# xinntao/EDVR

Hardware: AMD Instinct MI355X
Metric: EDVR-L x4 5-frame 720p clips/sec (higher is better)
Workload: dtype fp32 emulated as 2xf16 (hi+lo, 22-bit operands, 4 cross products), fp32 accumulate; 1 GPU; EDVR-L x4, 5 frames, 180x320 LR -> 720x1280, batch 10/GPU, inference; clips_per_gpu=10, global_clips=10, parallelism=clip-sharded x1, no data-path collective, world_size=1, backend=single process

## Files before the change

edvr_amd/_lib.py:

```python
import ctypes
import os

_HERE = os.path.dirname(os.path.abspath(__file__))
LIB_PATH = os.environ.get('EDVR_AMD_LIB') or os.path.join(_HERE, 'lib', 'libedvr_amd.so')

c_float_p = ctypes.c_void_p
i32, i64, f32, sz = ctypes.c_int, ctypes.c_int64, ctypes.c_float, ctypes.c_size_t
vp = ctypes.c_void_p


class ConvDesc(ctypes.Structure):
    _fields_ = [
        ('x1', vp), ('x2', vp), ('c1', i32), ('c2', i32), ('x1_img_stride', i64), ('x2_img_stride', i64),
        ('x2_div', i32), ('x2_mul', i32), ('x2_add', i32), ('n', i32), ('h', i32), ('w', i32), ('wpk', vp),
        ('bias', vp), ('co', i32), ('ks', i32), ('stride', i32), ('act', i32), ('act_from', i32), ('res1', vp),
        ('res2', vp), ('res1_img_stride', i64), ('res2_img_stride', i64), ('y', vp), ('y_img_stride', i64),
        ('out_mode', i32), ('algo', i32), ('gate', vp), ('gate_img_stride', i64), ('gate_slope', f32), ('y_scale', f32),
        ('wpk_f4', vp), ('abs_sum', vp), ('abs_sum_channels', i32), ('wpk_f4s', vp), ('x_amax', vp), ('y_amax', vp),
        ('pre', vp), ('pre_img_stride', i64), ('pre_div', i32), ('pre_mul', i32), ('pre_add', i32), ('pre_n', i32),
    ]


PROTOTYPES = {
    'edvr_version': (ctypes.c_char_p, []),
    'edvr_last_error': (ctypes.c_char_p, []),
    'edvr_check_device': (i32, []),
    'edvr_conv2d_packed_weight_elems': (sz, [i32, i32, i32]),
    'edvr_conv2d_pack_weight_f32': (i32, [vp, vp, i32, i32, i32, i32, vp]),
    'edvr_conv2d_packed_weight_f4_elems': (sz, [i32, i32]),
    'edvr_conv2d_pack_weight_f4_f32': (i32, [vp, vp, i32, i32, i32, vp]),
    'edvr_conv2d_packed_weight_f4s_elems': (sz, [i32, i32]),
    'edvr_conv2d_pack_weight_f4s_f32': (i32, [vp, vp, i32, i32, i32, vp]),
    'edvr_conv2d_packed_weight_1x1s_elems': (sz, [i32, i32]),
    'edvr_conv2d_pack_weight_1x1s_f32': (i32, [vp, vp, i32, i32, vp]),
    'edvr_amax_f32': (i32, [vp, vp, i32, i64, i64, vp]),
    'edvr_pack_job_bytes': (sz, []),
    'edvr_conv2d_pack_weights_multi': (i32, [vp, i32, i32, i32, vp]),
    'edvr_conv2d_f32': (i32, [ctypes.POINTER(ConvDesc), vp]),
    'edvr_conv2d_gate_supported': (i32, [ctypes.POINTER(ConvDesc)]),
    'edvr_conv2d_abs_sum_supported': (i32, [ctypes.POINTER(ConvDesc)]),
    'edvr_conv2d_y_amax_supported': (i32, [ctypes.POINTER(ConvDesc)]),
    'edvr_conv2d_pre_supported': (i32, [ctypes.POINTER(ConvDesc)]),
    'edvr_conv2d_kernel_name': (i32, [ctypes.POINTER(ConvDesc), ctypes.c_char_p, sz]),
    'edvr_conv2d_executed_flops': (i32, [ctypes.POINTER(ConvDesc), ctypes.POINTER(ctypes.c_double)]),
    'edvr_dcnv2_fwd_ws_bytes': (sz, [i32] * 12),
    'edvr_dcnv2_fwd_f32': (i32, [vp] * 6 + [i32] * 12 + [i64, i64, i32, i32, vp, sz, vp]),
    'edvr_dcnv2_fwd_split_f32': (i32, [vp] * 6 + [i32] * 12 + [i64, i64, i32, i32, vp, sz, vp, vp]),
    'edvr_dcnv2_fwd_split_applies': (i32, [vp] + [i32] * 13),
    'edvr_dcnv2_fwd_kernel_name': (i32, [vp] + [i32] * 13 + [ctypes.c_char_p, sz]),
    'edvr_dcnv2_bwd_ws_bytes': (sz, [i32] * 12),
    'edvr_dcnv2_any_ws_bytes': (sz, [i32] * 13),
    'edvr_dcnv2_fwd_any': (i32, [i32] + [vp] * 6 + [i32] * 12 + [i64, i64, vp, sz, vp]),
    'edvr_dcnv2_bwd_any': (i32, [i32] + [vp] * 10 + [i32] * 12 + [i64, i64, i64, i64, vp, sz, vp]),
    'edvr_psnr_sse_f32': (i32, [vp, vp, vp, i32, i32, i32, i32, i64, i64, i32, i32, i32, vp]),
    'edvr_ssim_partials': (sz, [i32, i32, i32]),
    'edvr_ssim_f32': (i32, [vp, vp, vp, i32, i32, i32, i32, i64, i64, i32, i32, vp]),
    'edvr_niqe_blocks': (sz, [i32, i32, i32]),
    'edvr_niqe_moments_f32': (i32, [vp, vp, i32, i32, i32, i32, i64, i32, vp]),
    'edvr_niqe_moments_u8': (i32, [vp, vp, i32, i32, i32, i64, i32, vp]),
    'edvr_frames_u8_to_f32': (i32, [vp, vp, i32, i32, i32, i32, vp, i32, vp]),
    'edvr_gather_images_f32': (i32, [vp, vp, vp, vp, i32, vp, i32, i32, vp]),
    'edvr_upsample4x_add_u8': (i32, [vp, vp, vp, i32, i32, i32, vp]),
    'edvr_f32_to_u8_hwc': (i32, [vp, vp, i32, i32, i32, i64, vp]),
    'edvr_crop_pad_frames_u8': (i32, [vp, vp, i32, i32, i32, i32, i32, i32, i32, i32, vp]),
    'edvr_crop_pad_frames_f32': (i32, [vp, vp, i32, i32, i32, i64, i32, i32, i32, i32, i32, vp]),
    'edvr_upsample4x_add_rect_f32': (i32, [vp, vp, vp, i32, i32, i32, i32, i32, i32, i32, i64, i64, i64, vp]),
    'edvr_upsample4x_add_rect_u8': (i32, [vp, vp, vp, i32, i32, i32, i32, i32, i32, i32, i64, i64, vp]),
    'edvr_f32_to_u8_hwc_rect': (i32, [vp, vp, i32, i32, i32, i64, i32, i32, i32, i32, i64, i64, vp]),
    'edvr_copy_rect_f32': (i32, [vp, vp, i32, i32, i32, i64, i32, i32, i32, i32, i64, i64, i64, vp]),
    'edvr_crop_pad_frames_d4_u8': (i32, [vp, vp, i32, i32, i32, i32, i32, i32, i32, i32, i32, vp]),
    'edvr_crop_pad_frames_d4_f32': (i32, [vp, vp, i32, i32, i32, i64, i32, i32, i32, i32, i32, i32, vp]),
    'edvr_upsample4x_add_rect_d4_f32': (i32, [vp, vp, vp, i32, i32, i32, i32, i32, i32, i32, i64, i64, i64, i32, i32, f32, vp]),
    'edvr_upsample4x_add_rect_d4_u8': (i32, [vp, vp, vp, vp, i32, i32, i32, i32, i32, i32, i32, i64, i64, i64, i64, i64, i32, i32, f32, vp]),
    'edvr_f32_to_u8_hwc_rect_d4': (i32, [vp, vp, vp, i32, i32, i32, i64, i32, i32, i32, i32, i64, i64, i64, i64, i64, i32, i32, f32, vp]),
    'edvr_copy_rect_d4_f32': (i32, [vp, vp, i32, i32, i32, i64, i32, i32, i32, i32, i64, i64, i64, i32, i32, f32, vp]),
    'edvr_upsample4x_add_rect_blend_f32': (i32, [vp, vp, vp, i32, i32, i32, i32, i32, i32, i32, i64, i64, i64, i32, i32, f32, i32, i32, i32, i32, vp]),
    'edvr_upsample4x_add_rect_blend_u8': (i32, [vp, vp, vp, vp, i32, i32, i32, i32, i32, i32, i32, i64, i64, i64, i64, i64, i32, i32, f32, i32, i32, i32, i32, vp]),
    'edvr_f32_to_u8_hwc_rect_blend': (i32, [vp, vp, vp, i32, i32, i32, i64, i32, i32, i32, i32, i64, i64, i64, i64, i64, i32, i32, f32, i32, i32, i32, i32, vp]),
    'edvr_copy_rect_blend_f32': (i32, [vp, vp, i32, i32, i32, i64, i32, i32, i32, i32, i64, i64, i64, i32, i32, f32, i32, i32, i32, i32, vp]),
    'edvr_imresize_bicubic_u8': (i32, [vp, vp, i32, i32, i32, i32, i32, ctypes.c_double, i32, i32, vp]),
    'edvr_imresize_bicubic_f32': (i32, [vp, vp, i32, i32, i32, i64, i32, i32, ctypes.c_double, i32, i32, vp]),
    'edvr_bd_downsample_u8': (i32, [vp, vp, i32, i32, i32, i32, i32, i32, i32, vp]),
    'edvr_bd_downsample_f32': (i32, [vp, vp, i32, i32, i32, i64, i32, i32, i32, i32, vp]),
    'edvr_imresize_bicubic_u8_windows': (i32, [vp, vp, vp, vp, i32, i32, i32, i32, i32, i32, vp]),
    'edvr_bd_downsample_u8_windows': (i32, [vp, vp, vp, vp, i32, i32, i32, i32, i32, i32, vp]),
    'edvr_yuv420_to_rgb_f32': (i32, [vp, vp, i32, i32, i32, i64, i64, vp, i32, vp]),
    'edvr_yuv420_to_rgb_u8': (i32, [vp, vp, i32, i32, i32, i64, vp, i32, vp]),
    'edvr_rgb_to_yuv420_f32': (i32, [vp, vp, i32, i32, i32, i64, i64, vp, vp]),
    'edvr_rgb_to_yuv420_u8': (i32, [vp, vp, i32, i32, i32, i64, vp, vp]),
    'edvr_adam_chunk_bytes': (sz, []),
    'edvr_adam_multi_f32': (i32, [vp, i32, ctypes.c_float, ctypes.c_float, ctypes.c_float, vp]),
    'edvr_dcnv1_fwd_ws_bytes': (sz, [i32] * 12),
    'edvr_dcnv1_fwd_f32': (i32, [vp] * 4 + [i32] * 12 + [i64, i32, vp, sz, vp]),
    'edvr_dcnv1_bwd_ws_bytes': (sz, [i32] * 12),
    'edvr_dcnv1_bwd_f32': (i32, [vp] * 7 + [i32] * 12 + [i64, i64, i32, vp, sz, vp]),
    'edvr_dcnv2_bwd_f32': (i32, [vp] * 10 + [i32] * 12 + [i64, i64, i64, i64, i32, vp, sz, vp]),
    'edvr_dcnv2_bwd_split_f32': (i32, [vp] * 10 + [i32] * 12 + [i64, i64, i64, i64, i32, vp, sz, vp, vp, vp]),
    'edvr_dcnv2_bwd_split_applies': (i32, []),
    'edvr_tsa_temporal_f32': (i32, [vp] * 5 + [i32] * 4 + [vp]),
    'edvr_tsa_temporal_pair_f32': (i32, [vp] * 5 + [i32] * 4 + [vp]),
    'edvr_pool_maxavg_3x3s2_f32': (i32, [vp, vp, i32, i32, i32, i32, vp]),
    'edvr_upsample2x_f32': (i32, [vp, vp, i32, i32, i32, f32, vp]),
    'edvr_tsa_combine_f32': (i32, [vp, vp, vp, vp, i64, vp]),
    'edvr_upsample4x_add_f32': (i32, [vp, vp, i32, i32, i32, vp]),
    'edvr_add_f32': (i32, [vp, vp, vp, i64, vp]),
    'edvr_act_bwd_f32': (i32, [vp, vp, vp, vp, vp, i32, i32, i64, i32, i32, vp]),
    'edvr_conv2d_wgrad_ws_bytes': (sz, [i32] * 7),
    'edvr_conv2d_wgrad_algo': (i32, [i32]),
    'edvr_conv2d_wgrad_kernel_name': (i32, [i32] * 8 + [ctypes.c_char_p, sz]),
    'edvr_conv2d_wgrad_f32': (i32, [vp] * 4 + [i32] * 8 + [i64, i64, i32, i32, i32, i64, i32, vp, vp, sz, vp]),
    'edvr_conv2d_wgrad_split_f32': (i32, [vp] * 4 + [i32] * 8 + [i64, i64, i32, i32, i32, i64, i32, vp, vp, sz, vp, vp, vp]),
    'edvr_conv2d_wgrad_split_applies': (i32, [i32] * 8),
    'edvr_conv2d_wgrad_split_is_direct': (i32, [i32] * 2),
    'edvr_channel_sum_f32': (i32, [vp, vp, i32, i32, i64, i64, vp, sz, vp]),
    'edvr_pixel_unshuffle2_f32': (i32, [vp, vp, i32, i32, i32, i32, vp]),
    'edvr_pixel_unshuffle2_act_bwd_f32': (i32, [vp, vp, vp, i32, i32, i32, i32, i32, vp]),
    'edvr_zero_stuff2_f32': (i32, [vp, vp, i32, i32, i32, i32, i32, vp]),
    'edvr_frame_reduce_add_f32': (i32, [vp, vp, i32, i32, i32, i64, vp]),
    'edvr_upsample2x_bwd_f32': (i32, [vp, vp, i32, i32, i32, f32, vp]),
    'edvr_pool_maxavg_3x3s2_bwd_f32': (i32, [vp, vp, vp, i32, i32, i32, i32, vp]),
    'edvr_tsa_temporal_bwd_f32': (i32, [vp] * 7 + [i32] * 4 + [vp, vp]),
    'edvr_tsa_combine_bwd_f32': (i32, [vp] * 5 + [i64, vp]),
    'edvr_charbonnier_f32': (i32, [vp, vp, vp, vp, i64, f32, f32, vp]),
    'edvr_abs_sum_f32': (i32, [vp, vp, i32, i64, i64, vp]),
    'edvr_abs_stats_f32': (i32, [vp, vp, i32, i64, i32, i64, vp]),
# ... 35 lines not shown
```

edvr_amd/csrc/winograd_f4s.hip:

```cpp
#include <cstdlib>
#include <type_traits>

#include "common.h"
#include "pack.h"

#ifndef F4S_PLAIN
#define F4S_PLAIN 1
#endif

namespace edvr {

typedef float f32x16 __attribute__((ext_vector_type(16)));
typedef float f32x4 __attribute__((ext_vector_type(4)));
typedef float f32x2 __attribute__((ext_vector_type(2)));
typedef int i32x4 __attribute__((ext_vector_type(4)));
typedef _Float16 f16x8 __attribute__((ext_vector_type(8)));

__device__ __forceinline__ float max_raw_s(float a, float b) {
  float o;
  asm("v_max_f32 %0, %1, %2" : "=v"(o) : "v"(a), "v"(b));
  return o;
}

__device__ __forceinline__ void split6_f16x2(const float (&x)[6], float s, unsigned (&o)[6]) {
  asm volatile(
      "v_fma_mixlo_f16 %0, %6, %12, 0\n\tv_fma_mixlo_f16 %1, %7, %12, 0\n\tv_fma_mixlo_f16 %2, %8, %12, 0\n\t"
      "v_fma_mixlo_f16 %3, %9, %12, 0\n\tv_fma_mixlo_f16 %4, %10, %12, 0\n\tv_fma_mixlo_f16 %5, %11, %12, 0\n\t"
      "v_fma_mixhi_f16 %0, %6, %12, -%0 op_sel_hi:[0,0,1]\n\tv_fma_mixhi_f16 %1, %7, %12, -%1 op_sel_hi:[0,0,1]\n\t"
      "v_fma_mixhi_f16 %2, %8, %12, -%2 op_sel_hi:[0,0,1]\n\tv_fma_mixhi_f16 %3, %9, %12, -%3 op_sel_hi:[0,0,1]\n\t"
      "v_fma_mixhi_f16 %4, %10, %12, -%4 op_sel_hi:[0,0,1]\n\tv_fma_mixhi_f16 %5, %11, %12, -%5 op_sel_hi:[0,0,1]"
      : "=&v"(o[0]), "=&v"(o[1]), "=&v"(o[2]), "=&v"(o[3]), "=&v"(o[4]), "=&v"(o[5])
      : "v"(x[0]), "v"(x[1]), "v"(x[2]), "v"(x[3]), "v"(x[4]), "v"(x[5]), "s"(s));
}

struct WinoF4SArgs {
  edvr_conv2d_desc d;
  const unsigned *U;
  int ci, ci_real, cop, tiles_x, tiles_y, items;
  float ys, ys_gs;
};

#define F4S_LDS_BARRIER() asm volatile("s_waitcnt lgkmcnt(0)\n\ts_barrier" ::: "memory")

#ifdef F4S_PROF
__device__ unsigned long long f4s_prof[16 * 8];
#define F4S_NOW(v) asm volatile("s_memtime %0\n\ts_waitcnt lgkmcnt(0)" : "=s"(v)::"memory")
#define F4S_BARRIER_AT(slot)                                        \
  do {                                                              \
    unsigned long long a_, b_;                                      \
    asm volatile("s_waitcnt lgkmcnt(0)" ::: "memory");              \
    F4S_NOW(a_);                                                    \
    asm volatile("s_barrier" ::: "memory");                         \
    F4S_NOW(b_);                                                    \
    f4s_pc[slot] += (unsigned)(b_ - a_);                            \
  } while (0)
#define F4S_SPAN_BEGIN() F4S_NOW(f4s_t0)
#define F4S_SPAN_END(slot)                                          \
  do {                                                              \
    unsigned long long b_;                                          \
    F4S_NOW(b_);                                                    \
    f4s_pc[slot] += (unsigned)(b_ - f4s_t0);                        \
    f4s_t0 = b_;                                                    \
  } while (0)
#define F4S_WAIT_DMA()                                              \
  do {                                                              \
    unsigned long long a_, b_;                                      \
    F4S_NOW(a_);                                                    \
    asm volatile("s_waitcnt vmcnt(0)" ::: "memory");                \
    F4S_NOW(b_);                                                    \
    f4s_pc[4] += (unsigned)(b_ - a_);                               \
  } while (0)
#define F4S_PROF_FLUSH()                                                                                         \
  do {                                                                                                          \
    if ((threadIdx.x & 63) == 0)                                                                                \
      for (int i_ = 0; i_ < 8; ++i_) atomicAdd(&f4s_prof[(threadIdx.x >> 6) * 8 + i_], (unsigned long long)f4s_pc[i_]); \
  } while (0)
#else
#define F4S_BARRIER_AT(slot) F4S_LDS_BARRIER()
#define F4S_SPAN_BEGIN()
#define F4S_SPAN_END(slot)
#define F4S_WAIT_DMA() asm volatile("s_waitcnt vmcnt(0)" ::: "memory")
#define F4S_PROF_FLUSH()
#endif
#if defined(F4S_PROF) && F4S_PROF >= 2
#define F4S_POS_T0() unsigned long long pa_, pb_, pc_; F4S_NOW(pa_)
#define F4S_POS_T1()                                                \
  do {                                                              \
    F4S_NOW(pb_);                                                   \
    asm volatile("s_waitcnt vmcnt(5)" ::: "memory");                \
    F4S_NOW(pc_);                                                   \
    f4s_pc[5] += (unsigned)(pb_ - pa_);                             \
    f4s_pc[6] += (unsigned)(pc_ - pb_);                             \
  } while (0)
#else
#define F4S_POS_T0()
#define F4S_POS_T1()
#endif
#define F4S_BARRIER() F4S_BARRIER_AT(7)

__device__ __forceinline__ float f4s_input_scale(float amax) {
  const int be = (int)((__builtin_bit_cast(unsigned, amax) >> 23) & 255u);
  const int field = min(max(127 + 8 - (be - 127), 7), 227);
  return __builtin_bit_cast(float, (unsigned)field << 23);
}

template <int TXL>
__global__ __launch_bounds__(1024, 1) void conv3x3_winograd_f4s_kernel(const WinoF4SArgs a) {
  constexpr int TX = 1 << TXL, TY = 32 / TX;
  constexpr int BW = 4 * TX, BH = 4 * TY;
  constexpr int RROWS = BH + 2, RPIECES = TX + 2;
  static_assert(RROWS * RPIECES == 180, "a wave's region holds 2 x 180 pieces either way");
  constexpr int CK = 8;
  constexpr int VSLAB = CK * 36 * 32;
  constexpr int XSZ = 2 * 6 * 8 * 32 * 4;
  constexpr int RWAVE = 6 * 64 * 4 + 4;
  constexpr int UCHUNK = 6 * 2 * 6 * 1024;
  __shared__ __attribute__((aligned(16))) float smem[2 * VSLAB + XSZ + 4 * RWAVE + 64];
  float *const Xs = smem + 2 * VSLAB;
  float *const bias_s = smem + 2 * VSLAB + XSZ + 4 * RWAVE;

  const edvr_conv2d_desc &d = a.d;
  const int tid = threadIdx.x, lane = tid & 63, half = lane >> 5, j = lane & 31;
// ... 146 lines not shown

    setup(item_first);
    load_begin(0);
    dma_issue();
    read_patch();
    advance();
    load_begin(l_k * CK);
    dma_issue();
#pragma unroll
    for (int cp = 0; cp < 3; ++cp) transform_cols(cp);
#pragma unroll
    for (int r = 0; r < 6; ++r) commit_row(Vst, r);
    F4S_BARRIER();

    int par = 0;
    float asum = 0.f;
    int asum_img = -1;
    auto asum_flush = [&]() {
      float s = asum;
#pragma unroll
      for (int sh = 32; sh > 0; sh >>= 1) s += __shfl_xor(s, sh);
      if (lane == 0 && asum_img >= 0 && s != 0.f) atomicAdd(d.abs_sum + asum_img, s);
      asum = 0.f;
    };
    unsigned amx = 0u;
    auto abits = [](float v) { return __builtin_bit_cast(unsigned, v) & 0x7fffffffu; };
    auto amax16 = [&](const f32x4 (&Y)[4], bool real) {
      unsigned m = 0u;
#pragma unroll
      for (int i = 0; i < 4; ++i) m = max(m, max(max(abits(Y[i][0]), abits(Y[i][1])), max(abits(Y[i][2]), abits(Y[i][3]))));
      amx = real ? max(amx, m) : amx;
    };
    F4S_SPAN_BEGIN();
    for (int item = item_first; item < item_end; item += xcd_wgs) {
      int e_co_blk, e_img, e_ty0, e_tx0;
      decode(item, e_co_blk, e_img, e_ty0, e_tx0);
      if (d.abs_sum && e_img != asum_img) {
        asum_flush();
        asum_img = e_img;
      }
#pragma unroll 1
      for (int k = 0; k < n_chunks; ++k) {
        unsigned *Vd = Vst + (par ^ 1) * VSLAB;
        read_patch();
        advance();
        load_begin(l_k * CK);
        dma_issue();
#pragma unroll
        for (int cp = 0; cp < 3; ++cp) transform_cols(cp);
#pragma unroll
        for (int r = 0; r < 6; ++r) commit_row(Vd, r);
        F4S_BARRIER_AT(0);
        par ^= 1;
      }
      F4S_SPAN_END(2);

      const int plane = hw;
      float *y = d.y + (int64_t)e_img * d.y_img_stride;
      const float *r1 = d.res1 ? d.res1 + (int64_t)e_img * d.res1_img_stride : nullptr;
      const float *r2 = d.res2 ? d.res2 + (int64_t)e_img * d.res2_img_stride : nullptr;
      const float *gt = d.gate ? d.gate + (int64_t)e_img * d.gate_img_stride : nullptr;
      const float *pq = nullptr;
      if (d.pre) pq = d.pre + (int64_t)(d.pre_div > 0 ? (e_img / d.pre_div) * d.pre_mul + d.pre_add : e_img) * d.pre_img_stride;
      const float *rq = gt ? gt : (pq ? pq : r1);
      const float slope = d.act == EDVR_ACT_LRELU ? 0.1f : (d.act == EDVR_ACT_RELU ? 0.f : 1.f);
      const bool sig = d.act == EDVR_ACT_SIGMOID, shuffle = d.out_mode == EDVR_OUT_PIXEL_SHUFFLE2;
      const bool vec = e_tx0 + BW <= d.w;
      const int cl8 = (wave * 64 + lane) >> 5, tile = lane & 31;
      const int oy = e_ty0 + 4 * (tile >> TXL), ox = e_tx0 + 4 * (tile & (TX - 1));
      const int co_t = e_co_blk + (cl8 >> 2) * 32 + 4 * ((cl8 >> 1) & 1) + 8 * (cl8 & 1);
      const int pix = oy * d.w + ox;
      const int rows_in = d.h - oy;
      if (wave == 0) bias_s[lane] = (d.bias && e_co_blk + lane < d.co) ? d.bias[e_co_blk + lane] : 0.f;
      auto column_pass = [&](auto VEC, auto SHUF, auto PREADD) {
        constexpr bool PRE = decltype(PREADD)::value;
        constexpr bool V = decltype(VEC)::value;
        constexpr bool SHF = decltype(SHUF)::value;
        f32x4 Yprev[4];
        f32x4 rr[4];
        auto co_of = [&](int p) { return co_t + (p & 3) + 16 * (p >> 2); };
        auto prefetch = [&](int p) {
          const int co = min(co_of(p), d.co - 1);
          if (V && !SHF && rq) {
            const float *q1 = rq + (int64_t)co * plane + pix;
#pragma unroll
            for (int i = 0; i < 4; ++i) rr[i] = i < rows_in ? *reinterpret_cast<const f32x4 *>(q1 + i * d.w) : f32x4{0.f, 0.f, 0.f, 0.f};
            if (r2) {
              const float *q2 = r2 + (int64_t)co * plane + pix;
#pragma unroll
              for (int i = 0; i < 4; ++i)
                if (i < rows_in) rr[i] += *reinterpret_cast<const f32x4 *>(q2 + i * d.w);
            }
          } else if (PRE && !V) {
            const float *q1 = pq + (int64_t)co * plane + pix;
#pragma unroll
            for (int i = 0; i < 4; ++i) rr[i] = (i < rows_in && ox < d.w) ? *reinterpret_cast<const f32x4 *>(q1 + i * d.w) : f32x4{0.f, 0.f, 0.f, 0.f};
          }
        };
        prefetch(0);
#pragma unroll 1
        for (int p = 0; p < 8; ++p) {
          F4S_BARRIER_AT(1);
          const float *Xb = Xs + (p & 1) * (XSZ / 2) + (cl8 * 32 + tile) * 4;
          f32x4 T[6];
#pragma unroll
          for (int r = 0; r < 6; ++r) T[r] = *reinterpret_cast<const f32x4 *>(Xb + r * (8 * 32 * 4));
          const int co = co_of(p);
          const float b = bias_s[co - e_co_blk];
          const float sl = co >= d.act_from ? slope : 1.f;
          f32x4 Y[4];
#pragma unroll
          for (int jp = 0; jp < 2; ++jp) {
            auto col2 = [&](int r) { return f32x2{T[r][2 * jp], T[r][2 * jp + 1]}; };
            const f32x2 t0 = col2(0), t1 = col2(1), t2 = col2(2), t3 = col2(3), t4 = col2(4), t5 = col2(5);
            const f32x2 s1 = t1 + t2, d1 = t1 - t2, s2 = t3 + t4, d2 = t3 - t4;
            const f32x2 us = f32x2{unscale, unscale}, bb = f32x2{b, b};
            f32x2 y0 = (t0 + s1 + s2) * us + bb;
            f32x2 y1 = (2.f * d2 + d1) * us + bb;
            f32x2 y2 = (4.f * s2 + s1) * us + bb;
            f32x2 y3 = (8.f * d2 + d1 + t5) * us + bb;
            if (PRE) {
              y0 += f32x2{rr[0][2 * jp], rr[0][2 * jp + 1]};
              y1 += f32x2{rr[1][2 * jp], rr[1][2 * jp + 1]};
              y2 += f32x2{rr[2][2 * jp], rr[2][2 * jp + 1]};
              y3 += f32x2{rr[3][2 * jp], rr[3][2 * jp + 1]};
            }
            if (!sig) {
              const f32x2 sl2 = f32x2{sl, sl};
              const f32x2 z0 = y0 * sl2, z1 = y1 * sl2, z2 = y2 * sl2, z3 = y3 * sl2;
              y0 = f32x2{max_raw_s(y0[0], z0[0]), max_raw_s(y0[1], z0[1])};
              y1 = f32x2{max_raw_s(y1[0], z1[0]), max_raw_s(y1[1], z1[1])};
              y2 = f32x2{max_raw_s(y2[0], z2[0]), max_raw_s(y2[1], z2[1])};
              y3 = f32x2{max_raw_s(y3[0], z3[0]), max_raw_s(y3[1], z3[1])};
            }
            Y[0][2 * jp] = y0[0]; Y[0][2 * jp + 1] = y0[1];
            Y[1][2 * jp] = y1[0]; Y[1][2 * jp + 1] = y1[1];
            Y[2][2 * jp] = y2[0]; Y[2][2 * jp + 1] = y2[1];
            Y[3][2 * jp] = y3[0]; Y[3][2 * jp + 1] = y3[1];
          }
          if (sig && co >= d.act_from) {
            if (d.y_amax) amx = max(amx, abits(__builtin_fmaf(Y[0][0], 0.f, __builtin_fmaf(Y[0][3], 0.f, __builtin_fmaf(Y[3][0], 0.f, Y[3][3] * 0.f)))));
            if (PRE && d.y_amax) {
#pragma unroll
              for (int i = 0; i < 4; ++i) amx = max(amx, abits(__builtin_fmaf(rr[i][0], 0.f, __builtin_fmaf(rr[i][1], 0.f, __builtin_fmaf(rr[i][2], 0.f, rr[i][3] * 0.f)))));
            }
#pragma unroll
            for (int i = 0; i < 4; ++i)
#pragma unroll
              for (int jj = 0; jj < 4; ++jj) Y[i][jj] = __builtin_amdgcn_rcpf(1.f + __expf(-Y[i][jj]));
          }
          if (SHF) {
            prefetch(min(p + 1, 7));
            if (d.y_amax) amax16(Y, co < d.co);
            if ((p & 1) == 0) {
#pragma unroll
              for (int i = 0; i < 4; ++i) Yprev[i] = Y[i];
            } else if (co < d.co) {
              float *q = y + (int64_t)(co >> 2) * plane * 4 + (2 * oy + ((co >> 1) & 1)) * (2 * d.w) + 2 * ox;
#pragma unroll
              for (int i = 0; i < 4; ++i)
                if (i < rows_in) {
                  *reinterpret_cast<f32x4 *>(q + i * 4 * d.w) = f32x4{Yprev[i][0], Y[i][0], Yprev[i][1], Y[i][1]};
                  *reinterpret_cast<f32x4 *>(q + i * 4 * d.w + 4) = f32x4{Yprev[i][2], Y[i][2], Yprev[i][3], Y[i][3]};
                }
            }
          } else if (V) {
            if (d.abs_sum && co < d.abs_sum_channels) {
#pragma unroll
              for (int i = 0; i < 4; ++i)
                if (i < rows_in) asum += (fabsf(Y[i][0]) + fabsf(Y[i][1])) + (fabsf(Y[i][2]) + fabsf(Y[i][3]));
            }
            if (gt) {
#pragma unroll
              for (int i = 0; i < 4; ++i)
#pragma unroll
                for (int jj = 0; jj < 4; ++jj) Y[i][jj] *= rr[i][jj] > 0.f ? a.ys : a.ys_gs;
            } else if (r1) {
#pragma unroll
              for (int i = 0; i < 4; ++i)
#pragma unroll
                for (int jj = 0; jj < 4; ++jj) Y[i][jj] = __builtin_fmaf(Y[i][jj], a.ys, rr[i][jj]);
            }
            prefetch(min(p + 1, 7));
            if (d.y_amax) amax16(Y, co < d.co);
            if (co < d.co) {
              float *q = y + (int64_t)co * plane + pix;
#pragma unroll
              for (int i = 0; i < 4; ++i)
                if (i < rows_in) *reinterpret_cast<f32x4 *>(q + i * d.w) = Y[i];
            }
          } else if (co < d.co) {
#pragma unroll 1
            for (int i = 0; i < 4; ++i) {
              if (oy + i >= d.h) break;
              const int64_t off = (int64_t)co * plane + pix + i * d.w;
#pragma unroll
              for (int jj = 0; jj < 4; ++jj) {
                if (ox + jj < d.w) {
                  float o = Y[i][jj];
                  if (d.abs_sum && co < d.abs_sum_channels) asum += fabsf(o);
                  if (gt) o *= gt[off + jj] > 0.f ? a.ys : a.ys_gs;
                  else if (r1) o = __builtin_fmaf(o, a.ys, r1[off + jj] + (r2 ? r2[off + jj] : 0.f));
                  amx = max(amx, abits(o));
                  if (shuffle)
                    y[(int64_t)(co >> 2) * plane * 4 + (2 * (oy + i) + ((co >> 1) & 1)) * (2 * d.w) + 2 * (ox + jj) + (co & 1)] = o;
                  else
                    y[off + jj] = o;
                }
              }
            }
            prefetch(min(p + 1, 7));
          } else {
            prefetch(min(p + 1, 7));
          }
        }
      };
      if (pq && vec) column_pass(std::true_type{}, std::false_type{}, std::true_type{});
      else if (pq) column_pass(std::false_type{}, std::false_type{}, std::true_type{});
      else if (vec && shuffle) column_pass(std::true_type{}, std::true_type{}, std::false_type{});
      else if (vec) column_pass(std::true_type{}, std::false_type{}, std::false_type{});
      else column_pass(std::false_type{}, std::false_type{}, std::false_type{});
      F4S_SPAN_END(3);
    }
    if (d.abs_sum) asum_flush();
    if (d.y_amax) {
#pragma unroll
      for (int sh = 32; sh > 0; sh >>= 1) amx = max(amx, (unsigned)__shfl_xor((int)amx, sh));
      if (lane == 0 && amx > 0u) atomicMax(reinterpret_cast<unsigned *>(d.y_amax), amx);
    }
    F4S_PROF_FLUSH();
  } else {
    const int q = wave - 4, wm = q & 1, row = q >> 1;
    const __amdgpu_buffer_rsrc_t u_rsrc = uniform_rsrc(a.U, 64 + a.cop * a.ci * 36 * 4);
    const int voff = lane * 16;
    f32x16 acc[6];
    i32x4 A[6];
    int u_base = 0, u_next = 0;
    auto item_base = [&](int co_blk) { return 64 + ((((co_blk >> 6) * n_chunks) * 6 + row) * 2 + wm) * (6 * 1024); };
    auto load_a = [&](int c, int soff) { A[c] = __builtin_bit_cast(i32x4, __builtin_amdgcn_raw_buffer_load_b128(u_rsrc, voff, soff + c * 1024, 0)); };
    int co_blk, img_, ty_, tx_;
    decode(item_first, co_blk, img_, ty_, tx_);
    u_base = item_base(co_blk);
#pragma unroll
    for (int c = 0; c < 6; ++c) load_a(c, u_base);
#pragma unroll
    for (int c = 0; c < 6; ++c)
#pragma unroll
      for (int r = 0; r < 16; ++r) acc[c][r] = 0.f;
    F4S_BARRIER();

    int par = 0;
    const unsigned *const Vst = reinterpret_cast<const unsigned *>(smem);
    unsigned v_addr = (unsigned)(size_t)(__attribute__((address_space(3))) const unsigned *)(Vst + 4 * half * 36 * 32 + row * 6 * 32 + j);
    int v_step = __builtin_amdgcn_readfirstlane(VSLAB * 4);
    F4S_SPAN_BEGIN();
    for (int item = item_first; item < item_end; item += xcd_wgs) {
      {
        const int nx = item + xcd_wgs;
        decode(nx < item_end ? nx : item, co_blk, img_, ty_, tx_);
        u_next = item_base(co_blk);
      }
#pragma unroll 1
      for (int k = 0; k < n_chunks; ++k) {
        const int soff_nxt = k + 1 < n_chunks ? u_base + (k + 1) * UCHUNK : u_next;
#pragma unroll
        for (int c = 0; c < 6; ++c) {
          int b0, b1, b2, b3;
          F4S_POS_T0();
          asm volatile("ds_read_b32 %0, %4 offset:%5\n\tds_read_b32 %1, %4 offset:%6\n\tds_read_b32 %2, %4 offset:%7\n\tds_read_b32 %3, %4 offset:%8\n\t"
                       "s_waitcnt lgkmcnt(0)"
                       : "=&v"(b0), "=&v"(b1), "=&v"(b2), "=&v"(b3)
                       : "v"(v_addr), "n"(c * 128), "n"(36 * 128 + c * 128), "n"(2 * 36 * 128 + c * 128), "n"(3 * 36 * 128 + c * 128)
                       : "memory");
          F4S_POS_T1();
          const f16x8 B = __builtin_bit_cast(f16x8, i32x4{b0, b1, b2, b3});
          acc[c] = __builtin_amdgcn_mfma_f32_32x32x16_f16(__builtin_bit_cast(f16x8, A[c]), B, acc[c], 0, 0, 0);
          asm volatile("v_alignbit_b32 %0, %0, %0, 16\n\tv_alignbit_b32 %1, %1, %1, 16\n\tv_alignbit_b32 %2, %2, %2, 16\n\tv_alignbit_b32 %3, %3, %3, 16"
                       : "+v"(A[c][0]), "+v"(A[c][1]), "+v"(A[c][2]), "+v"(A[c][3]));
          acc[c] = __builtin_amdgcn_mfma_f32_32x32x16_f16(__builtin_bit_cast(f16x8, A[c]), B, acc[c], 0, 0, 0);
          __builtin_amdgcn_sched_barrier(0);
          load_a(c, soff_nxt);
          __builtin_amdgcn_sched_barrier(0);
        }
        v_addr += v_step;
        v_step = -v_step;
        F4S_BARRIER_AT(0);
        par ^= 1;
      }
      u_base = u_next;
      F4S_SPAN_END(2);
      int lane_e = lane;
      asm volatile("" : "+v"(lane_e));
      float *const Xw = Xs + ((row * 8 + wm * 4 + (lane_e >> 5) * 2) * 32 + (lane_e & 31)) * 4;
#pragma unroll
      for (int p = 0; p < 8; ++p) {
        float *Xb = Xw + (p & 1) * (XSZ / 2);
#pragma unroll
        for (int rr = 0; rr < 2; ++rr) {
          const int r = (p & 3) + 4 * (2 * (p >> 2) + rr);
          const float m0 = acc[0][r], m1 = acc[1][r], m2 = acc[2][r], m3 = acc[3][r], m4 = acc[4][r], m5 = acc[5][r];
// ... 32 lines not shown
    const unsigned field = f4s_weight_scale_field(__builtin_bit_cast(unsigned, m));
    U[0] = field << 23;
    U[1] = (254u - field) << 23;
    for (int i = 2; i < 16; ++i) U[i] = 0u;
  }
}

__global__ void winograd_f4s_weight_kernel(const float *__restrict__ w, unsigned *__restrict__ U, int co, int ci, int cop, int cip, int transpose_flip) {
  const int64_t total = (int64_t)cip * cop;
  const float s_u = __builtin_bit_cast(float, U[0]);
  for (int64_t i = (int64_t)blockIdx.x * blockDim.x + threadIdx.x; i < total; i += (int64_t)gridDim.x * blockDim.x)
    pack_f4s_elem(w, U, i, co, ci, cop, cip, transpose_flip, s_u);
}

__global__ __launch_bounds__(256) void amax_kernel(const float *__restrict__ x, unsigned *__restrict__ out, int n, int64_t per_img, int64_t img_stride) {
  unsigned m = 0u;
  auto ab = [](float v) { return __builtin_bit_cast(unsigned, v) & 0x7fffffffu; };
  auto ab4 = [&](const f32x4 &v) { return max(max(ab(v[0]), ab(v[1])), max(ab(v[2]), ab(v[3]))); };
  const int64_t quads = per_img >> 2;
  const int64_t step = (int64_t)gridDim.x * 256;
  for (int img = blockIdx.y; img < n; img += gridDim.y) {
    const float *p = x + (int64_t)img * img_stride;
    if ((reinterpret_cast<uintptr_t>(p) & 15) == 0) {
      const f32x4 *q = reinterpret_cast<const f32x4 *>(p);
      int64_t i = (int64_t)blockIdx.x * 256 + threadIdx.x;
      for (; i + 3 * step < quads; i += 4 * step) {
        const f32x4 a = q[i], b = q[i + step], c = q[i + 2 * step], e = q[i + 3 * step];
        m = max(m, max(max(ab4(a), ab4(b)), max(ab4(c), ab4(e))));
      }
      for (; i < quads; i += step) m = max(m, ab4(q[i]));
      for (int64_t t = quads * 4 + (int64_t)blockIdx.x * 256 + threadIdx.x; t < per_img; t += step) m = max(m, ab(p[t]));
    } else {
      for (int64_t t = (int64_t)blockIdx.x * 256 + threadIdx.x; t < per_img; t += step) m = max(m, ab(p[t]));
    }
  }
#pragma unroll
  for (int sh = 32; sh > 0; sh >>= 1) m = max(m, (unsigned)__shfl_xor((int)m, sh));
  if ((threadIdx.x & 63) == 0 && m > 0u) atomicMax(out, m);
}

bool winograd_f4s_enabled() {
  static const bool on = []() {
    const char *e = getenv("EDVR_WINOGRAD_F4S");
    const char *w = getenv("EDVR_CONV_WINOGRAD");
    return !(e && e[0] == '0') && !(w && w[0] == '0');
  }();
  return on;
}

bool winograd_f4s_supported(const edvr_conv2d_desc &d) {
  if (!d.wpk_f4s || !d.x_amax || d.ks != 3 || d.stride != 1) return false;
  const bool has_res = d.res1 || d.res2;
  if (d.gate && (has_res || d.act == EDVR_ACT_SIGMOID || d.out_mode != EDVR_OUT_NCHW)) return false;
  if ((d.res2 && !d.res1) || (d.out_mode != EDVR_OUT_NCHW && has_res)) return false;
  if (d.pre && (d.gate || has_res || d.out_mode != EDVR_OUT_NCHW)) return false;
  if (d.y_scale != 0.f && d.y_scale != 1.f && !d.res1 && !d.gate) return false;
  if (d.c2 > 0 && (d.c1 & 1)) return false;
  if ((int64_t)((d.co + 63) / 64 * 64) * ((d.c1 + d.c2 + 7) / 8 * 8) * 144 + 64 >= ((int64_t)1 << 31)) return false;
  if ((int64_t)d.h * d.w * 8 >= ((int64_t)1 << 31)) return false;
  if (d.w & 3) return false;
  auto aligned = [](const void *p, int64_t img_stride, int a) { return !p || ((reinterpret_cast<uintptr_t>(p) & (a - 1)) == 0 && (img_stride * 4 & (a - 1)) == 0); };
  if (!aligned(d.x1, d.x1_img_stride, 16) || !aligned(d.x2, d.x2_img_stride, 16)) return false;
  if (!aligned(d.y, d.y_img_stride, 16) || !aligned(d.res1, d.res1_img_stride, 16) || !aligned(d.res2, d.res2_img_stride, 16) ||
      !aligned(d.gate, d.gate_img_stride, 16) || !aligned(d.wpk_f4s, 0, 16) || !aligned(d.pre, d.pre_img_stride, 16))
    return false;
  return true;
}

bool winograd_f4s_eligible(const edvr_conv2d_desc &d) {
  if (!winograd_f4s_supported(d)) return false;
  if (d.algo == EDVR_CONV_WINOGRAD_F4S) return true;
  if (d.algo != EDVR_CONV_AUTO || !winograd_f4s_enabled()) return false;
  return d.co >= 48 && d.c1 + d.c2 >= 32 && d.w >= 32 && d.h >= 8;
}

static int f4s_geometry(const edvr_conv2d_desc &d, int &tiles_x, int &tiles_y, bool &tx8) {
  const int64_t pad16 = (int64_t)cdiv(d.w, 64) * 64 * cdiv(d.h, 8) * 8, pad8 = (int64_t)cdiv(d.w, 32) * 32 * cdiv(d.h, 16) * 16;
  tx8 = pad8 < pad16;
  tiles_x = cdiv(d.w, tx8 ? 32 : 64);
  tiles_y = cdiv(d.h, tx8 ? 16 : 8);
  return tiles_x * tiles_y * cdiv(d.co, 64) * d.n;
}

double winograd_f4s_executed_flops(const edvr_conv2d_desc &d) {
  int tx, ty;
  bool tx8;
  const double items = f4s_geometry(d, tx, ty, tx8);
  return items * ((d.c1 + d.c2 + 7) / 8) * 144.0 * 32768.0;
}

int winograd_f4s_launch(const edvr_conv2d_desc &d, hipStream_t stream) {
  WinoF4SArgs a;
  a.d = d;
  a.U = reinterpret_cast<const unsigned *>(d.wpk_f4s);
  a.ci_real = d.c1 + d.c2;
  a.ci = (a.ci_real + 7) / 8 * 8;
  a.cop = (d.co + 63) / 64 * 64;
  a.ys = d.y_scale == 0.f ? 1.f : d.y_scale;
  a.ys_gs = a.ys * d.gate_slope;
  bool tx8;
  a.items = f4s_geometry(d, a.tiles_x, a.tiles_y, tx8);
  static const int n_cu = []() {
    int dev = 0, n = 256;
    hipDeviceProp_t prop;
    if (hipGetDevice(&dev) == hipSuccess && hipGetDeviceProperties(&prop, dev) == hipSuccess) n = prop.multiProcessorCount;
    return n;
  }();
  const dim3 grid(std::min(a.items, n_cu));
  if (tx8) hipLaunchKernelGGL(conv3x3_winograd_f4s_kernel<3>, grid, dim3(1024), 0, stream, a);
  else hipLaunchKernelGGL(conv3x3_winograd_f4s_kernel<4>, grid, dim3(1024), 0, stream, a);
  return check_launch("conv3x3_winograd_f4s_kernel");
}

}

extern "C" {

#ifdef F4S_PROF
int edvr_f4s_prof_read(unsigned long long *host, int reset) {
  int rc = (int)hipMemcpyFromSymbol(host, HIP_SYMBOL(edvr::f4s_prof), sizeof(unsigned long long) * 128);
  if (rc == 0 && reset) {
    static unsigned long long zero[128];
    rc = (int)hipMemcpyToSymbol(HIP_SYMBOL(edvr::f4s_prof), zero, sizeof(zero));
  }
  return rc;
}
#endif

size_t edvr_conv2d_packed_weight_f4s_elems(int co, int ci) { return 16 + (size_t)((co + 63) / 64 * 64) * ((ci + 7) / 8 * 8) * 36; }

int edvr_conv2d_pack_weight_f4s_f32(const float *w, void *wpk_f4s, int co, int ci, int transpose_flip, edvr_stream_t stream) {
  EDVR_REQUIRE(w && wpk_f4s && co > 0 && ci > 0, "pack_weight_f4s: bad arguments");
  const int cop = (co + 63) / 64 * 64, cip = (ci + 7) / 8 * 8;
  const int64_t total = (int64_t)cip * cop;
  unsigned *U = reinterpret_cast<unsigned *>(wpk_f4s);
  hipLaunchKernelGGL(edvr::winograd_f4s_weight_scale_kernel, dim3(1), dim3(1024), 0, edvr::as_stream(stream), w, U, (int64_t)co * ci * 9);
  hipLaunchKernelGGL(edvr::winograd_f4s_weight_kernel, dim3((unsigned)std::min<int64_t>(edvr::cdiv64(total, 256), 4096)), dim3(256), 0,
                     edvr::as_stream(stream), w, U, co, ci, cop, cip, transpose_flip);
  return edvr::check_launch("winograd_f4s_weight_kernel");
}

int edvr_amax_f32(const float *x, float *amax, int n, int64_t per_img, int64_t img_stride, edvr_stream_t stream) {
  EDVR_REQUIRE(x && amax && n > 0 && per_img > 0, "amax: bad arguments");
  if (img_stride == per_img || n == 1) {
    per_img *= n;
    n = 1;
  }
  const int bx = (int)std::min<int64_t>(edvr::cdiv64(per_img, 256 * 16), 2048);
  const int by = std::min(n, std::max(1, 2048 / bx));
  hipLaunchKernelGGL(edvr::amax_kernel, dim3(bx, by), dim3(256), 0, edvr::as_stream(stream), x, reinterpret_cast<unsigned *>(amax), n, per_img,
                     img_stride);
  return edvr::check_launch("amax_kernel");
}

}
```

include/edvr_amd.h:

```cpp
#ifndef EDVR_AMD_H
#define EDVR_AMD_H

#include <stddef.h>
#include <stdint.h>

#ifdef __cplusplus
extern "C" {
#endif

#define EDVR_OK 0
#define EDVR_ERR_ARG (-1)
#define EDVR_ERR_UNSUPPORTED (-2)
#define EDVR_ERR_LAUNCH (-3)
#define EDVR_ERR_WORKSPACE (-4)

typedef void *edvr_stream_t;

const char *edvr_version(void);
const char *edvr_last_error(void);
int edvr_check_device(void);

#define EDVR_ACT_NONE 0
#define EDVR_ACT_RELU 1
#define EDVR_ACT_LRELU 2
#define EDVR_ACT_SIGMOID 3

#define EDVR_DCN_HALO_TAPWIN 16
#define EDVR_DCN_SCATTER_AUTO 0
#define EDVR_DCN_SCATTER_DEVICE 1
#define EDVR_DCN_SCATTER_LDS 2
#define EDVR_DCN_SCATTER_STRIP 3
#define EDVR_DCN_SCATTER_LDS_WIDE 4
#define EDVR_CONV_AUTO 0
#define EDVR_CONV_DIRECT 1
#define EDVR_CONV_WINOGRAD 2
#define EDVR_CONV_WINOGRAD_F4 3
#define EDVR_CONV_WINOGRAD_F4S 4

#define EDVR_OUT_NCHW 0
#define EDVR_OUT_PIXEL_SHUFFLE2 1

typedef struct edvr_conv2d_desc {
  const float *x1;
  const float *x2;
  int c1, c2;
  int64_t x1_img_stride;
  int64_t x2_img_stride;
  int x2_div, x2_mul, x2_add;
  int n, h, w;
  const float *wpk;
  const float *bias;
  int co, ks, stride;
  int act;
  int act_from;
  const float *res1;
  const float *res2;
  int64_t res1_img_stride, res2_img_stride;
  float *y;
  int64_t y_img_stride;
  int out_mode;
  int algo;
  const float *gate;
  int64_t gate_img_stride;
  float gate_slope;
  float y_scale;
  const float *wpk_f4;
  float *abs_sum;
  int abs_sum_channels;
  const void *wpk_f4s;
  const float *x_amax;
  float *y_amax;
  const float *pre;
  int64_t pre_img_stride;
  int pre_div, pre_mul, pre_add;
  int pre_n;
} edvr_conv2d_desc;

size_t edvr_conv2d_packed_weight_elems(int co, int ci, int ks);
int edvr_conv2d_pack_weight_f32(const float *w, float *wpk, int co, int ci, int ks, int transpose_flip,
                                edvr_stream_t stream);
size_t edvr_conv2d_packed_weight_f4_elems(int co, int ci);
int edvr_conv2d_pack_weight_f4_f32(const float *w, float *wpk_f4, int co, int ci, int transpose_flip, edvr_stream_t stream);
size_t edvr_conv2d_packed_weight_f4s_elems(int co, int ci);
int edvr_conv2d_pack_weight_f4s_f32(const float *w, void *wpk_f4s, int co, int ci, int transpose_flip, edvr_stream_t stream);
size_t edvr_conv2d_packed_weight_1x1s_elems(int co, int ci);
int edvr_conv2d_pack_weight_1x1s_f32(const float *w, void *wpk_1x1s, int co, int ci, edvr_stream_t stream);
int edvr_amax_f32(const float *x, float *amax, int n, int64_t per_img, int64_t img_stride, edvr_stream_t stream);
size_t edvr_pack_job_bytes(void);
int edvr_conv2d_pack_weights_multi(const void *jobs, int n_jobs, int total_blocks, int split_parity, edvr_stream_t stream);
int edvr_conv2d_f32(const edvr_conv2d_desc *d, edvr_stream_t stream);
int edvr_conv2d_gate_supported(const edvr_conv2d_desc *d);
int edvr_conv2d_y_amax_supported(const edvr_conv2d_desc *d);
int edvr_conv2d_abs_sum_supported(const edvr_conv2d_desc *d);
int edvr_conv2d_pre_supported(const edvr_conv2d_desc *d);
int edvr_conv2d_kernel_name(const edvr_conv2d_desc *d, char *buf, size_t buf_len);
int edvr_conv2d_executed_flops(const edvr_conv2d_desc *d, double *flops);

#define EDVR_HW(h, w) ((int)(h) | (((int)(w) + 1) << 16))

size_t edvr_dcnv2_fwd_ws_bytes(int B, int C, int H, int W, int Co, int kh, int kw, int stride, int pad, int dil,
                               int groups, int dg);
int edvr_dcnv2_fwd_f32(const float *x, const float *offset, const float *mask, const float *weight,
                       const float *bias, float *y, int B, int C, int H, int W, int Co, int kh, int kw, int stride,
                       int pad, int dil, int groups, int dg, int64_t offset_bstride, int64_t mask_bstride, int act,
                       int halo_hint, void *ws, size_t ws_bytes, edvr_stream_t stream);

int edvr_dcnv2_fwd_split_f32(const float *x, const float *offset, const float *mask, const float *weight, const float *bias,
                             float *y, int B, int C, int H, int W, int Co, int kh, int kw, int stride, int pad, int dil, int groups,
                             int dg, int64_t offset_bstride, int64_t mask_bstride, int act, int halo_hint, void *ws, size_t ws_bytes,
                             const float *xm_amax, edvr_stream_t stream);
int edvr_dcnv2_fwd_split_applies(const float *x, int B, int C, int H, int W, int Co, int kh, int kw, int stride, int pad, int dil, int groups,
                                 int dg, int halo_hint);
int edvr_dcnv2_fwd_kernel_name(const float *x, int B, int C, int H, int W, int Co, int kh, int kw, int stride, int pad, int dil,
                               int groups, int dg, int halo_hint, char *buf, size_t buf_len);

size_t edvr_dcnv2_bwd_ws_bytes(int B, int C, int H, int W, int Co, int kh, int kw, int stride, int pad, int dil,
                               int groups, int dg);
int edvr_dcnv2_bwd_f32(const float *x, const float *offset, const float *mask, const float *weight, const float *dy,
                       float *dx, float *doffset, float *dmask, float *dweight, float *dbias, int B, int C, int H,
                       int W, int Co, int kh, int kw, int stride, int pad, int dil, int groups, int dg,
                       int64_t offset_bstride, int64_t mask_bstride, int64_t doffset_bstride, int64_t dmask_bstride,
                       int scatter_hint, void *ws, size_t ws_bytes, edvr_stream_t stream);
int edvr_dcnv2_bwd_split_f32(const float *x, const float *offset, const float *mask, const float *weight, const float *dy,
                             float *dx, float *doffset, float *dmask, float *dweight, float *dbias, int B, int C, int H,
                             int W, int Co, int kh, int kw, int stride, int pad, int dil, int groups, int dg,
                             int64_t offset_bstride, int64_t mask_bstride, int64_t doffset_bstride, int64_t dmask_bstride,
                             int scatter_hint, void *ws, size_t ws_bytes, const float *xm_amax, const float *dy_amax,
                             edvr_stream_t stream);
int edvr_dcnv2_bwd_split_applies(void);

#define EDVR_DTYPE_F32 0
#define EDVR_DTYPE_F64 1
#define EDVR_DTYPE_F16 2
size_t edvr_dcnv2_any_ws_bytes(int dtype, int B, int C, int H, int W, int Co, int kh, int kw, int stride, int pad, int dil, int groups,
                               int dg);
int edvr_dcnv2_fwd_any(int dtype, const void *x, const void *offset, const void *mask, const void *weight, const void *bias, void *y, int B,
                       int C, int H, int W, int Co, int kh, int kw, int stride, int pad, int dil, int groups, int dg,
                       int64_t offset_bstride, int64_t mask_bstride, void *ws, size_t ws_bytes, edvr_stream_t stream);
int edvr_dcnv2_bwd_any(int dtype, const void *x, const void *offset, const void *mask, const void *weight, const void *dy, void *dx,
                       void *doffset, void *dmask, void *dweight, void *dbias, int B, int C, int H, int W, int Co, int kh, int kw, int stride,
                       int pad, int dil, int groups, int dg, int64_t offset_bstride, int64_t mask_bstride, int64_t doffset_bstride,
                       int64_t dmask_bstride, void *ws, size_t ws_bytes, edvr_stream_t stream);

size_t edvr_dcnv1_fwd_ws_bytes(int B, int C, int H, int W, int Co, int kh, int kw, int stride, int pad, int dil,
                               int groups, int dg);
int edvr_dcnv1_fwd_f32(const float *x, const float *offset, const float *weight, float *y, int B, int C, int H, int W,
                       int Co, int kh, int kw, int stride, int pad, int dil, int groups, int dg, int64_t offset_bstride,
                       int halo_hint, void *ws, size_t ws_bytes, edvr_stream_t stream);
size_t edvr_dcnv1_bwd_ws_bytes(int B, int C, int H, int W, int Co, int kh, int kw, int stride, int pad, int dil,
                               int groups, int dg);
int edvr_dcnv1_bwd_f32(const float *x, const float *offset, const float *weight, const float *dy, float *dx,
                       float *doffset, float *dweight, int B, int C, int H, int W, int Co, int kh, int kw, int stride,
                       int pad, int dil, int groups, int dg, int64_t offset_bstride, int64_t doffset_bstride,
                       int scatter_hint, void *ws, size_t ws_bytes, edvr_stream_t stream);

int edvr_tsa_temporal_f32(const float *emb, const float *emb_ref, const float *aligned, float *out, float *prob_out,
                          int b, int t, int c, int hw, edvr_stream_t stream);
int edvr_tsa_temporal_pair_f32(const float *emb, const float *emb_ref, const float *aligned, float *out, float *out_rev,
                               int b, int t, int c, int hw, edvr_stream_t stream);
int edvr_pool_maxavg_3x3s2_f32(const float *x, float *y, int n, int c, int h, int w, edvr_stream_t stream);
int edvr_upsample2x_f32(const float *x, float *y, int nc, int h, int w, float scale, edvr_stream_t stream);
int edvr_tsa_combine_f32(const float *feat, const float *attn, const float *attn_add, float *y, int64_t numel,
                         edvr_stream_t stream);
int edvr_upsample4x_add_f32(const float *base, float *y, int nc, int h, int w, edvr_stream_t stream);
int edvr_add_f32(const float *a, const float *b, float *y, int64_t numel, edvr_stream_t stream);
int edvr_act_bwd_f32(const float *dy, const float *y, const float *res1, const float *res2, float *dz, int n, int c,
                     int64_t hw, int act, int act_from, edvr_stream_t stream);
int edvr_abs_sum_f32(const float *x, float *out, int n, int64_t per_img, int64_t img_stride, edvr_stream_t stream);
int edvr_abs_stats_f32(const float *x, float *out, int n, int64_t per_img, int w, int64_t img_stride, edvr_stream_t stream);

size_t edvr_conv2d_wgrad_ws_bytes(int n, int ci, int h, int w, int co, int ks, int stride);
int edvr_conv2d_wgrad_f32(const float *x1, const float *x2, const float *dz, float *dw, int c1, int c2, int n, int h, int w,
                          int co, int ks, int stride, int64_t x1_img_stride, int64_t x2_img_stride, int x2_div, int x2_mul,
                          int x2_add, int64_t dz_img_stride, int accumulate, float *dbias, void *ws, size_t ws_bytes,
                          edvr_stream_t stream);
int edvr_conv2d_wgrad_split_f32(const float *x1, const float *x2, const float *dz, float *dw, int c1, int c2, int n, int h, int w,
                                int co, int ks, int stride, int64_t x1_img_stride, int64_t x2_img_stride, int x2_div, int x2_mul,
// ... 127 lines not shown
```

Before: 99.96 clips/s.

## Add lean Winograd F4 epilogue path for full interior output tiles

Adds a specialised output-transform/epilogue for the F4S Winograd conv, used on items whose tile and 64-channel block are fully in bounds. It uses buffer-resource loads and stores with precomputed offsets, compile-time activation and residual/pre-add variants, and an integer-bit amax reduction, which removes the per-element bounds checks and generic branching of the existing column pass. It is on by default and can be turned off with an env var or an API toggle; there is also a small waitcnt tweak in the old prefetch. The cost is more code variants and higher register and instruction-cache pressure.

New measurement: 101.5 clips/s (median of 6 runs). +1.6%, better.

```diff
diff --git a/edvr_amd/_lib.py b/edvr_amd/_lib.py
--- a/edvr_amd/_lib.py
+++ b/edvr_amd/_lib.py
@@ -41,6 +41,8 @@
     'edvr_conv2d_abs_sum_supported': (i32, [ctypes.POINTER(ConvDesc)]),
     'edvr_conv2d_y_amax_supported': (i32, [ctypes.POINTER(ConvDesc)]),
     'edvr_conv2d_pre_supported': (i32, [ctypes.POINTER(ConvDesc)]),
+    'edvr_conv2d_f4s_set_lean': (i32, [i32]),
+    'edvr_conv2d_f4s_lean_items': (i32, [ctypes.POINTER(ConvDesc)]),
     'edvr_conv2d_kernel_name': (i32, [ctypes.POINTER(ConvDesc), ctypes.c_char_p, sz]),
     'edvr_conv2d_executed_flops': (i32, [ctypes.POINTER(ConvDesc), ctypes.POINTER(ctypes.c_double)]),
     'edvr_dcnv2_fwd_ws_bytes': (sz, [i32] * 12),
diff --git a/edvr_amd/csrc/winograd_f4s.hip b/edvr_amd/csrc/winograd_f4s.hip
--- a/edvr_amd/csrc/winograd_f4s.hip
+++ b/edvr_amd/csrc/winograd_f4s.hip
@@ -1,3 +1,4 @@
+#include <atomic>
 #include <cstdlib>
 #include <type_traits>
 
@@ -38,6 +39,7 @@
   const unsigned *U;
   int ci, ci_real, cop, tiles_x, tiles_y, items;
   float ys, ys_gs;
+  int lean;
 };
 
 #define F4S_LDS_BARRIER() asm volatile("s_waitcnt lgkmcnt(0)\n\ts_barrier" ::: "memory")
@@ -350,6 +352,7 @@
         auto prefetch = [&](int p) {
           const int co = min(co_of(p), d.co - 1);
           if (V && !SHF && rq) {
+            if (!PRE) __builtin_amdgcn_s_waitcnt(0x0f70);
             const float *q1 = rq + (int64_t)co * plane + pix;
 #pragma unroll
             for (int i = 0; i < 4; ++i) rr[i] = i < rows_in ? *reinterpret_cast<const f32x4 *>(q1 + i * d.w) : f32x4{0.f, 0.f, 0.f, 0.f};
@@ -483,7 +486,107 @@
           }
         }
       };
-      if (pq && vec) column_pass(std::true_type{}, std::false_type{}, std::true_type{});
+      int lean_f = a.lean, pb = plane_bytes, w4 = d.w * 4;
+      asm volatile("" : "+s"(lean_f), "+s"(pb), "+s"(w4));
+      const bool lean_item = (lean_f & 1) && vec && e_ty0 + BH <= d.h && e_co_blk + 64 <= d.co && (!(lean_f & 4) || d.act_from <= e_co_blk);
+      auto column_pass_lean = [&](auto ACT_, auto ADD_) {
+        constexpr bool ACT = decltype(ACT_)::value;
+        constexpr int ADD = decltype(ADD_)::value;
+        const int64_t blk = (int64_t)e_co_blk * (pb >> 2);
+        const __amdgpu_buffer_rsrc_t y_rs = uniform_rsrc(y + blk, 64 * pb);
+        const __amdgpu_buffer_rsrc_t q_rs = uniform_rsrc(ADD ? (ADD == 2 ? pq : r1) + blk : y, ADD ? 64 * pb : 0);
+        int voff[4];
+#pragma unroll
+        for (int i = 0; i < 4; ++i) voff[i] = (co_t - e_co_blk) * pb + pix * 4 + i * w4;
+        float us1 = unscale, sl1 = slope, ys1 = a.ys;
+        asm volatile("" : "+v"(us1), "+v"(sl1), "+v"(ys1));
+        const f32x2 us = f32x2{us1, us1}, sl2 = f32x2{sl1, sl1};
+        const bool want_amax = (lean_f & 2) != 0;
+        const float *bp = bias_s + (co_t - e_co_blk);
+        const float *Xb = Xs + (cl8 * 32 + tile) * 4;
+        int x_step = XSZ / 2;
+        int soff = 0;
+        int pmax = 0;
+        unsigned umax = 0u;
+        f32x4 rr[4];
+        if (ADD) {
+#pragma unroll
+          for (int i = 0; i < 4; ++i) rr[i] = __builtin_bit_cast(f32x4, __builtin_amdgcn_raw_buffer_load_b128(q_rs, voff[i], 0, 0));
+        }
+#pragma unroll 1
+        for (int p = 0; p < 8; ++p) {
+          F4S_BARRIER_AT(1);
+          f32x4 T[6];
+#pragma unroll
+          for (int r = 0; r < 6; ++r) T[r] = *reinterpret_cast<const f32x4 *>(Xb + r * (8 * 32 * 4));
+          const float b = *bp;
+          f32x4 Y[4];
+#pragma unroll
+          for (int jp = 0; jp < 2; ++jp) {
+            auto col2 = [&](int r) { return f32x2{T[r][2 * jp], T[r][2 * jp + 1]}; };
+            const f32x2 t0 = col2(0), t1 = col2(1), t2 = col2(2), t3 = col2(3), t4 = col2(4), t5 = col2(5);
+            const f32x2 s1 = t1 + t2, d1 = t1 - t2, s2 = t3 + t4, d2 = t3 - t4;
+            const f32x2 bb = f32x2{b, b};
+            f32x2 y0 = (t0 + s1 + s2) * us + bb;
+            f32x2 y1 = (2.f * d2 + d1) * us + bb;
+            f32x2 y2 = (4.f * s2 + s1) * us + bb;
+            f32x2 y3 = (8.f * d2 + d1 + t5) * us + bb;
+            if (ADD == 2) {
+              y0 += f32x2{rr[0][2 * jp], rr[0][2 * jp + 1]};
+              y1 += f32x2{rr[1][2 * jp], rr[1][2 * jp + 1]};
+              y2 += f32x2{rr[2][2 * jp], rr[2][2 * jp + 1]};
+              y3 += f32x2{rr[3][2 * jp], rr[3][2 * jp + 1]};
+            }
+            if (ACT) {
+              const f32x2 z0 = y0 * sl2, z1 = y1 * sl2, z2 = y2 * sl2, z3 = y3 * sl2;
+              y0 = f32x2{max_raw_s(y0[0], z0[0]), max_raw_s(y0[1], z0[1])};
+              y1 = f32x2{max_raw_s(y1[0], z1[0]), max_raw_s(y1[1], z1[1])};
+              y2 = f32x2{max_raw_s(y2[0], z2[0]), max_raw_s(y2[1], z2[1])};
+              y3 = f32x2{max_raw_s(y3[0], z3[0]), max_raw_s(y3[1], z3[1])};
+            }
+            Y[0][2 * jp] = y0[0]; Y[0][2 * jp + 1] = y0[1];
+            Y[1][2 * jp] = y1[0]; Y[1][2 * jp + 1] = y1[1];
+            Y[2][2 * jp] = y2[0]; Y[2][2 * jp + 1] = y2[1];
+            Y[3][2 * jp] = y3[0]; Y[3][2 * jp + 1] = y3[1];
+          }
+          if (ADD == 1) {
+#pragma unroll
+            for (int i = 0; i < 4; ++i)
+#pragma unroll
+              for (int jj = 0; jj < 4; ++jj) Y[i][jj] = __builtin_fmaf(Y[i][jj], ys1, rr[i][jj]);
+          }
+#pragma unroll
+          for (int i = 0; i < 4; ++i) __builtin_amdgcn_raw_buffer_store_b128(__builtin_bit_cast(i32x4, Y[i]), y_rs, voff[i], soff, 0);
+          soff += (p & 3) == 3 ? 13 * pb : pb;
+          bp += (p & 3) == 3 ? 13 : 1;
+          Xb += x_step;
+          x_step = -x_step;
+          if (ADD && p != 7) {
+#pragma unroll
+            for (int i = 0; i < 4; ++i) rr[i] = __builtin_bit_cast(f32x4, __builtin_amdgcn_raw_buffer_load_b128(q_rs, voff[i], soff, 0));
+          }
+          if (want_amax) {
+#pragma unroll
+            for (int i = 0; i < 4; ++i) {
+              const i32x4 yb = __builtin_bit_cast(i32x4, Y[i]);
+              pmax = max(max(pmax, yb[0]), yb[1]);
+              pmax = max(max(pmax, yb[2]), yb[3]);
+              umax = max(max(umax, (unsigned)yb[0]), (unsigned)yb[1]);
+              umax = max(max(umax, (unsigned)yb[2]), (unsigned)yb[3]);
+            }
+          }
+        }
+        amx = max(amx, max((unsigned)max(pmax, 0), umax & 0x7fffffffu));
+      };
+      if (lean_item) {
+        auto with_add = [&](auto ACT_) {
+          if (lean_f & 16) column_pass_lean(ACT_, std::integral_constant<int, 2>{});
+          else if (lean_f & 8) column_pass_lean(ACT_, std::integral_constant<int, 1>{});
+          else column_pass_lean(ACT_, std::integral_constant<int, 0>{});
+        };
+        if (lean_f & 4) with_add(std::true_type{});
+        else with_add(std::false_type{});
+      } else if (pq && vec) column_pass(std::true_type{}, std::false_type{}, std::true_type{});
       else if (pq) column_pass(std::false_type{}, std::false_type{}, std::true_type{});
       else if (vec && shuffle) column_pass(std::true_type{}, std::true_type{}, std::false_type{});
       else if (vec) column_pass(std::true_type{}, std::false_type{}, std::false_type{});
@@ -682,6 +785,39 @@
   return tiles_x * tiles_y * cdiv(d.co, 64) * d.n;
 }
 
+static std::atomic<int> &f4s_lean_switch() {
+  static std::atomic<int> on([]() {
+    const char *e = getenv("EDVR_F4S_LEAN");
+    return (e && e[0] == '0') ? 0 : 1;
+  }());
+  return on;
+}
+
+static int f4s_lean_launch(const edvr_conv2d_desc &d) {
+  if (!f4s_lean_switch().load(std::memory_order_relaxed)) return 0;
+  if (d.out_mode != EDVR_OUT_NCHW || d.gate || d.abs_sum || d.res2) return 0;
+  if (d.act != EDVR_ACT_NONE && d.act != EDVR_ACT_RELU && d.act != EDVR_ACT_LRELU) return 0;
+  if ((int64_t)d.h * d.w * 4 * 64 >= ((int64_t)1 << 31)) return 0;
+  return 1 | (d.y_amax ? 2 : 0) | (d.act != EDVR_ACT_NONE ? 4 : 0) | (d.pre ? 16 : (d.res1 ? 8 : 0));
+}
+
+static bool f4s_lean_item(const edvr_conv2d_desc &d, int co_blk, int ty0, int tx0, int bw, int bh) {
+  return tx0 + bw <= d.w && ty0 + bh <= d.h && co_blk + 64 <= d.co && (d.act == EDVR_ACT_NONE || d.act_from <= co_blk);
+}
+
+int winograd_f4s_lean_items(const edvr_conv2d_desc &d) {
+  if (!f4s_lean_launch(d)) return 0;
+  int tiles_x, tiles_y;
+  bool tx8;
+  f4s_geometry(d, tiles_x, tiles_y, tx8);
+  const int bw = tx8 ? 32 : 64, bh = tx8 ? 16 : 8;
+  int per_img = 0;
+  for (int cb = 0; cb < d.co; cb += 64)
+    for (int ty = 0; ty < tiles_y; ++ty)
+      for (int tx = 0; tx < tiles_x; ++tx) per_img += f4s_lean_item(d, cb, ty * bh, tx * bw, bw, bh) ? 1 : 0;
+  return per_img * d.n;
+}
+
 double winograd_f4s_executed_flops(const edvr_conv2d_desc &d) {
   int tx, ty;
   bool tx8;
@@ -700,6 +836,7 @@
   a.ys_gs = a.ys * d.gate_slope;
   bool tx8;
   a.items = f4s_geometry(d, a.tiles_x, a.tiles_y, tx8);
+  a.lean = f4s_lean_launch(d);
   static const int n_cu = []() {
     int dev = 0, n = 256;
     hipDeviceProp_t prop;
@@ -726,6 +863,15 @@
   return rc;
 }
 #endif
+
+int edvr_conv2d_f4s_set_lean(int on) { return edvr::f4s_lean_switch().exchange(on ? 1 : 0); }
+
+int edvr_conv2d_f4s_lean_items(const edvr_conv2d_desc *d) {
+  if (!d) return 0;
+  const bool scaled = d->y_scale != 0.f && d->y_scale != 1.f;
+  if ((!d->gate && !scaled && edvr::conv_small_eligible(*d)) || !edvr::winograd_f4s_eligible(*d)) return 0;
+  return edvr::winograd_f4s_lean_items(*d);
+}
 
 size_t edvr_conv2d_packed_weight_f4s_elems(int co, int ci) { return 16 + (size_t)((co + 63) / 64 * 64) * ((ci + 7) / 8 * 8) * 36; }
 
diff --git a/include/edvr_amd.h b/include/edvr_amd.h
--- a/include/edvr_amd.h
+++ b/include/edvr_amd.h
@@ -93,6 +93,8 @@
 int edvr_conv2d_y_amax_supported(const edvr_conv2d_desc *d);
 int edvr_conv2d_abs_sum_supported(const edvr_conv2d_desc *d);
 int edvr_conv2d_pre_supported(const edvr_conv2d_desc *d);
+int edvr_conv2d_f4s_set_lean(int on);
+int edvr_conv2d_f4s_lean_items(const edvr_conv2d_desc *d);
 int edvr_conv2d_kernel_name(const edvr_conv2d_desc *d, char *buf, size_t buf_len);
 int edvr_conv2d_executed_flops(const edvr_conv2d_desc *d, double *flops);
 
```
